# kazuotani14/iLQR

Measured on AMD Instinct MI355X. Metric: iLQR iterations/sec (batch x T timesteps/sec), acrobot T=500 batch=4096, higher is better.
Workload: dtype f64; 1 GPU; acrobot n=4 m=1 T=499 (500 knots), box-QP limits active, FD derivatives + backward/box-QP + 11-alpha search + accept, fixed work; batch_per_gpu=4096, global_batch=4096, T=499, parallelism=batch shards x1, one all_gather of costs

## Files before the change

### ilqr_amd/csrc/backward_hex.hpp

```cpp
#pragma once
#include "solve_tile.hpp"

namespace ilqr {

#ifndef ILQR_COMMIT_ROLLED
#define ILQR_COMMIT_ROLLED 1
#endif

#ifndef ILQR_COMMIT_BATCH
#define ILQR_COMMIT_BATCH 2
#endif
constexpr int kCommitBatch = ILQR_COMMIT_BATCH;

constexpr int HT = 4;
#ifndef ILQR_HEX_SLOT_PAD
#define ILQR_HEX_SLOT_PAD 8
#endif
#ifndef ILQR_HEX_PAIR_PERM
#define ILQR_HEX_PAIR_PERM 1
#endif
#ifndef ILQR_HEX_CAND_T
#define ILQR_HEX_CAND_T 1
#endif
constexpr bool kHexCandT = ILQR_HEX_CAND_T != 0;
#ifndef ILQR_HEX_QUAD_ROLLOUT
#define ILQR_HEX_QUAD_ROLLOUT 1
#endif
constexpr bool kHexQuadRollout = ILQR_HEX_QUAD_ROLLOUT != 0;

template <int NX, int NU, class real, int SLOTS_, bool COMPACT_ = false>
struct HexRing {
  static constexpr bool COMPACT = COMPACT_;
  static constexpr int US = Rec<NX, NU>::SIZE;
  static constexpr int PAIRS = COMPACT ? CompactRec<NX, NU>::PAIRS : (Rec<NX, NU>::SIZE + NU + 1) / 2;
  static constexpr int ROW = 2 * HT;
  static constexpr int PAD = ROW - 2 * TW;
  static constexpr int ELEMS = PAIRS * ROW + ILQR_HEX_SLOT_PAD;
  static constexpr int Z = PAIRS * ROW;
  static_assert(!COMPACT || ILQR_HEX_SLOT_PAD >= ROW, "the compact slot keeps Z in its pad row");
  static_assert(!COMPACT || (NX == 4 && NU == 1), "compact slots: nx = 4, nu = 1");
  static constexpr int SLOTS = SLOTS_;
  static constexpr bool PERM = (ILQR_HEX_PAIR_PERM != 0) && NX == 4 && NU == 1;
  static constexpr int pos(int pair) { return PERM && (!COMPACT || pair < 8) ? hex_pair_pos(pair) : pair; }
};

constexpr int kHexKnotsPerRound = 64 / HT;
constexpr int kHexFullSlots = 24;
template <int NX, int NU, class real, bool COMPACT>
struct HexRingSize {
  using Full = HexRing<NX, NU, real, kHexFullSlots, false>;
  static constexpr int TERM = COMPACT ? ((NX + NX * NX) / 2) * Full::ROW : 0;
  static constexpr int SLOTS = COMPACT ? (kHexFullSlots * Full::ELEMS - TERM) / HexRing<NX, NU, real, 1, COMPACT>::ELEMS : kHexFullSlots;
  static constexpr int LEAD = SLOTS - kHexKnotsPerRound - 1;
  static_assert(SLOTS > LEAD + kHexKnotsPerRound - 1 && LEAD >= 1, "a round must not reach a slot the chain has not left");
  static_assert(SLOTS * HexRing<NX, NU, real, 1, COMPACT>::ELEMS + TERM <= kHexFullSlots * Full::ELEMS, "the pair's records fit the bytes of 24 full slots");
};

template <class real, int N>
struct HexTerm {
  alignas(16) real term[N];
};
template <class real>
struct HexTerm<real, 0> {
  static constexpr real* term = nullptr;
};

template <class real, int NX, int NU, bool COMPACT = false>
struct HexPair : HexTerm<real, HexRingSize<NX, NU, real, COMPACT>::TERM> {
  using Size = HexRingSize<NX, NU, real, COMPACT>;
  using RS = HexRing<NX, NU, real, Size::SLOTS, COMPACT>;
  static constexpr int LEAD = Size::LEAD;
  alignas(16) real ring[RS::SLOTS * RS::ELEMS];
  int rounds_done;
  int consumer_at;
  int passes_started;
  unsigned long long pass_lanes;
};

template <class P>
struct HexGate {
  static constexpr bool kRing = true;
  P& sh;
  const int T, nrounds, N;
  int pass = -1, have = 0;
  int g_next = 0, slot_next = 0, slot_cur = 0;
  __device__ __forceinline__ HexGate(P& s, int T_) : sh(s), T(T_), nrounds((T_ + 1 + kHexKnotsPerRound - 1) / kHexKnotsPerRound), N(nrounds * kHexKnotsPerRound) {}
  __device__ __forceinline__ void begin_pass() {
    pass++;
    have = pass * N;
    g_next = pass * N;
    slot_next = g_next % P::RS::SLOTS;
    __hip_atomic_store(&sh.pass_lanes, __ballot(1), __ATOMIC_RELAXED, __HIP_MEMORY_SCOPE_WORKGROUP);
    __hip_atomic_store(&sh.passes_started, pass + 1, __ATOMIC_RELEASE, __HIP_MEMORY_SCOPE_WORKGROUP);
  }
  __device__ __forceinline__ int slot(int) const { return slot_cur; }
  __device__ __forceinline__ void wait(int) {
    const int G = g_next++;
    slot_cur = slot_next;
    slot_next = (slot_next + 1 == P::RS::SLOTS) ? 0 : slot_next + 1;
    __hip_atomic_store(&sh.consumer_at, G, __ATOMIC_RELAXED, __HIP_MEMORY_SCOPE_WORKGROUP);
    if (G < have) return;
    const int round = pass * nrounds + (G - pass * N) / kHexKnotsPerRound;
    while (__hip_atomic_load(&sh.rounds_done, __ATOMIC_ACQUIRE, __HIP_MEMORY_SCOPE_WORKGROUP) <= round) __builtin_amdgcn_s_sleep(1);
    have = pass * N + ((G - pass * N) / kHexKnotsPerRound + 1) * kHexKnotsPerRound;
  }
  __device__ __forceinline__ void finish() {
    __hip_atomic_store(&sh.consumer_at, 0x3fffffff, __ATOMIC_RELAXED, __HIP_MEMORY_SCOPE_WORKGROUP);
    __hip_atomic_store(&sh.passes_started, -1, __ATOMIC_RELEASE, __HIP_MEMORY_SCOPE_WORKGROUP);
  }
};

__device__ __forceinline__ int hex_first(unsigned long long bal, int t4) {
  return __builtin_ctzll(((bal >> t4) & 0x000F000F000F000Full) | 0x8000000000000000ull);
}
__device__ __forceinline__ void qp1_search_hex(QP1StateT<double>& q, int j, int t4, double step_j0, const double* __restrict__ lds_steps) {
  const double t_x1 = clamp_of(q.x + step_j0 * q.search, q.lo, q.hi);
  const double t_v1 = qp1_value(q, t_x1);
  const bool t_pass = !qp1_armijo_fails(q, t_v1, step_j0);
  const int pp = hex_first(__ballot(t_pass), t4);
  const bool success = pp < 52;
  const int jw = success ? (((pp >> 4) << 2) | (pp & 3)) : 0;
#ifdef ILQR_EXP_NO_STEP_LDS
  q.step = jw == 0 ? 1.0 : 0.6;
#else
  q.step = lds_steps[jw];
#endif
  q.x1 = clamp_of(q.x + q.step * q.search, q.lo, q.hi);
  q.v1 = qp1_value(q, q.x1);
  bool more = p_and(!success, !q.early);
  if (__builtin_expect(__ballot(more) == 0ull, 1)) return;
  {
    const bool stuck = p_and(j >= 1, t_x1 == q.x);
    const int qs = hex_first(__ballot(p_and(stuck, more)), t4);
    if (p_and(more, qs < 52)) {
      q.ls_failed = true;
      more = false;
    }
    if (__ballot(more) == 0ull) return;
  }
  for (int base = 16;; base += 16) {
    const int kn = base + j;
    const double my_step = lds_steps[kn < 104 ? kn : 103];
    const double my_x1 = qp1_trial(q, my_step);
    const double my_v1 = qp1_value(q, my_x1);
    const bool pass = !qp1_armijo_fails(q, my_v1, my_step);
    const bool stuck = p_or(my_step < kMinStep, my_x1 == q.x);
    const int qp = hex_first(__ballot(p_and(pass, more)), t4), qs = hex_first(__ballot(p_and(stuck, more)), t4);
    if (more) {
      if (qp < qs) {
        q.step = lds_steps[base + (((qp >> 4) << 2) | (qp & 3))];
        q.x1 = qp1_trial(q, q.step);
        q.v1 = qp1_value(q, q.x1);
        more = false;
      } else if (qs < 52) {
        q.ls_failed = true;
        more = false;
      }
    }
    if (__ballot(more) == 0ull) return;
  }
}

template <class RS>
__device__ __forceinline__ int hex_pos_rt(int pair) { return RS::pos(pair); }

template <class real>
struct HexStep {
  typedef real pair_t __attribute__((ext_vector_type(2)));
  real F, cxx_rc, cxx_cr, fu_r, cx_r, cxu_r, cxu_c;
  pair_t tail, uw;
};

template <class M, class Gate, class RS>
__device__ __forceinline__ void backward_hex(const BatchViewT<typename M::real>& v, const M& model, const SolverParams& sp, int mode, int tile, int sub,
                                             int lane, const double* __restrict__ lds_steps, Gate& gate, const typename M::real* __restrict__ ring,
                                             const typename M::real* __restrict__ term ) {
  using real = typename M::real;
  using creal = double;
  static_assert(M::NX == 4 && M::NU == 1, "hex chain: nx = 4, nu = 1");
  using R = Rec<4, 1>;
  typedef real real2_t __attribute__((ext_vector_type(2)));
  const int r_ = lane >> 4, t_ = (lane >> 2) & 3, c_ = lane & 3, j16 = 4 * r_ + c_;
  const int t4 = 4 * t_;
  const int l = sub * HT + t_;
  const int b = tile * TW + l;
  if (b >= v.B) return;
  if (mode == 1 && v.status[b] != 0) return;
  const int T = v.T;
  double lambda = v.lambda[b], dlambda = v.dlambda[b];
  const real* __restrict__ ust = v.us + tidx(tile, 0, 0, l, T, 1);
  real* __restrict__ kt = v.kff + tidx(tile, 0, 0, l, T, 1);
  real* __restrict__ Kt = v.Kfb + tidx(tile, 0, 0, l, T, 4);
  typedef const __attribute__((address_space(3))) real lds_cd;
  typedef const __attribute__((address_space(3))) real2_t lds_cd2;
  const creal step_j0 = lds_steps[j16];
  auto mm = [](creal a, creal bb) __attribute__((always_inline)) { return __builtin_amdgcn_mfma_f64_4x4x4f64(a, bb, 0.0, 0, 0, 0); };

  auto load = [&](int t, HexStep<real>& d) __attribute__((always_inline)) {
    gate.wait(t);
    lds_cd* r = (lds_cd*)(ring + gate.slot(t) * RS::ELEMS + t_ * 2);
    auto pair = [&](int e) { return *(lds_cd2*)(r + RS::pos(e >> 1) * RS::ROW); };
    auto one = [&](int e) { return r[hex_pos_rt<RS>(e >> 1) * RS::ROW + (e & 1)]; };
    if constexpr (RS::COMPACT) {
      using C = CompactRec<4, 1>;
      d.F = one(C::FX + r_ + 4 * c_);
      d.fu_r = one(C::FU + r_);
      d.cxx_rc = d.cxx_cr = d.cx_r = d.cxu_r = d.cxu_c = r[RS::Z];
      d.tail = pair(C::CU);
      d.uw = pair(C::US);
      return;
    }
    d.F = one(R::FX + r_ + 4 * c_);
    d.cxx_rc = one(R::CXX + r_ + 4 * c_);
    d.cxx_cr = one(R::CXX + c_ + 4 * r_);
    d.fu_r = one(R::FU + r_);
    d.cx_r = one(R::CX + r_);
    d.cxu_r = one(R::CXU + r_);
    d.cxu_c = one(R::CXU + c_);
    d.tail = pair(R::CU);
    d.uw = pair(RS::US);
  };

  int diverge = 0;
  bool done = false;
  double dV0 = 0, dV1 = 0, gacc = 0;
  auto one_pass = [&]() __attribute__((always_inline)) {
    gate.begin_pass();
    creal V, RVx, kprev;
    const creal lam_r = (creal)lambda;
    {
      gate.wait(T);
      if constexpr (RS::COMPACT) {
        using C = CompactRec<4, 1>;
        lds_cd* r = (lds_cd*)(term + t_ * 2);
        RVx = (creal)r[((C::TERM_CX + r_) >> 1) * RS::ROW + ((C::TERM_CX + r_) & 1)];
        V = (creal)r[((C::TERM_CXX + r_ + 4 * c_) >> 1) * RS::ROW + ((C::TERM_CXX + r_ + 4 * c_) & 1)];
      } else {
      lds_cd* r = (lds_cd*)(ring + gate.slot(T) * RS::ELEMS + t_ * 2);
      RVx = (creal)r[hex_pos_rt<RS>((R::CX + r_) >> 1) * RS::ROW + ((R::CX + r_) & 1)];
      V = (creal)r[hex_pos_rt<RS>((R::CXX + r_ + 4 * c_) >> 1) * RS::ROW + ((R::CXX + r_ + 4 * c_) & 1)];
      }
    }
    kprev = (creal)kt[(unsigned)((T - 1) * TW)];
    __builtin_amdgcn_s_waitcnt(0x0F70);
    dV0 = dV1 = 0;
    diverge = 0;
    gacc = 0;
    real* __restrict__ Kt_i = Kt + (unsigned)(((T - 1) * 4 + c_) * TW);
    real* __restrict__ kt_i = kt + (unsigned)((T - 1) * TW);

    auto step = [&](int i, const HexStep<real>& raw, HexStep<real>& nxt) -> bool {
      const creal F = (creal)raw.F, Rfu = (creal)raw.fu_r;
      const creal cu = (creal)raw.tail.x, cuu = (creal)raw.tail.y, us = (creal)raw.uw.x, usw = (creal)raw.uw.y;
      const creal W = mm(V, F);
      const creal wv = mm(V, Rfu);
      const creal aQu = mm(Rfu, RVx);
      const creal aQx = mm(F, RVx);
      const creal Tm = mm(F, W);
      const creal Tt = mm(W, F);
      const creal aQuu = mm(Rfu, wv);
      const creal aQux_c = mm(Rfu, W);
      const creal aQux_r = mm(W, Rfu);
      const creal Qxx_rc = (creal)raw.cxx_rc + Tm, Qxx_cr = (creal)raw.cxx_cr + Tt;
      const creal Qx_r = (creal)raw.cx_r + aQx;
      const creal Qu = cu + aQu;
      const creal Qux_c = (creal)raw.cxu_c + aQux_c, Qux_r = (creal)raw.cxu_r + aQux_r;
      const creal Quu = cuu + aQuu, QuuF = (cuu + lam_r) + aQuu;
      const creal lo = (creal)model.u_min[0] - us, hi = (creal)model.u_max[0] - us;
      __builtin_amdgcn_sched_barrier(0);
      if (i >= 1) load(i - 1, nxt);
      __builtin_amdgcn_sched_barrier(0);
      creal x;
      int free0;
      creal minv;
      QP1StateT<creal> q1;
      qp1_begin<false>(QuuF, Qu, kprev, lo, hi, q1, false);
      qp1_search_hex(q1, j16, t4, step_j0, lds_steps);
      bool goes_on;
      bool ok = qp1_finish_ok(q1, x, free0, minv, goes_on);
      if (goes_on)
        ok = qp1_continue(
                 q1, [&](QP1StateT<creal>& qs) __attribute__((always_inline)) { qp1_search_hex(qs, j16, t4, step_j0, lds_steps); }, x, free0) >= 1;
      if (!ok) diverge = i;
      const creal k_scale = free0 ? -minv : creal(0);
      const creal K_r = k_scale * Qux_r, K_c = k_scale * Qux_c;
      creal d0 = 0, d1 = 0;
      {
        d0 += x * Qu;
        creal rq = 0;
        rq += (creal(0.5) * x) * Quu;
        d1 += rq * x;
      }
      creal T1_r, T1_c;
      {
        creal acc = 0;
        acc += K_r * Quu;
        T1_r = acc;
      }
      {
        creal acc = 0;
        acc += K_c * Quu;
        T1_c = acc;
      }
      creal Vxn_r, Vn_rc, Vn_cr;
      {
        creal t1 = 0, t2 = 0, t3 = 0;
        t1 += T1_r * x;
        t2 += K_r * Qu;
        t3 += Qux_r * x;
        Vxn_r = ((Qx_r + t1) + t2) + t3;
      }
      {
        creal u1 = 0, u2 = 0, u3 = 0;
        u1 += T1_r * K_c;
        u2 += K_r * Qux_c;
        u3 += Qux_r * K_c;
        Vn_rc = ((Qxx_rc + u1) + u2) + u3;
      }
      {
        creal u1 = 0, u2 = 0, u3 = 0;
        u1 += T1_c * K_r;
        u2 += K_c * Qux_r;
        u3 += Qux_c * K_r;
        Vn_cr = ((Qxx_cr + u1) + u2) + u3;
      }
      V = creal(0.5) * (Vn_rc + Vn_cr);
      RVx = Vxn_r;
      if (ok) {
        dV0 += (double)d0;
        dV1 += (double)d1;
        gacc += (double)(abs_of(x) * usw);
        kprev = (creal)(real)x;
        Kt_i[0] = (real)K_c;
        kt_i[0] = (real)x;
      }
      Kt_i -= 4 * TW;
      kt_i -= TW;
      return ok;
    };

    HexStep<real> A, Bd;
    int i = T - 1;
    load(i, A);
    while (true) {
      if (!step(i, A, Bd)) break;
      if (--i < 0) break;
      if (!step(i, Bd, A)) break;
      if (--i < 0) break;
    }
  };

  while (true) {
    one_pass();
    if (mode == 0) {
      done = (diverge == 0);
      break;
    }
    if (diverge != 0) {
      dlambda = raised_dlambda(dlambda, sp);
      lambda = raised_lambda(lambda, dlambda, sp);
      if (lambda > sp.lambda_max) break;
      continue;
    }
    done = true;
    break;
  }

  double acc = gacc;
  if (!done) {
    __builtin_amdgcn_fence(__ATOMIC_RELEASE, "workgroup");
    __builtin_amdgcn_s_waitcnt(0);
    acc = 0;
    for (int t0 = 0; t0 < T; t0 += 8) {
      real kv[8], uv[8];
#pragma unroll
      for (int jj = 0; jj < 8; jj++) {
        const int t = (t0 + jj < T) ? t0 + jj : T - 1;
        kv[jj] = kt[(size_t)t * TW];
        uv[jj] = ust[(size_t)t * TW];
      }
#pragma unroll
      for (int jj = 0; jj < 8; jj++) {
        const real mx = abs_of(kv[jj]) / (abs_of(uv[jj]) + 1);
        if (t0 + jj < T) acc += (double)mx;
      }
    }
  }
  const double gnorm = acc / T;
  if (j16 == 0) {
    v.dV[b] = dV0;
    v.dV[v.Bp + b] = dV1;
    v.diverge[b] = diverge;
    v.backpass_done[b] = done ? 1 : 0;
    v.gnorm[b] = gnorm;
    if (mode == 1) {
      v.lambda[b] = lambda;
      v.dlambda[b] = dlambda;
      if (!sp.fixed_work && gnorm < sp.tol_grad && lambda < kLambdaConverged) {
        v.status[b] = 1;
        v.iters[b] += 1;
      }
    }
  }
}

template <class M, class MFD, class P>
__device__ __forceinline__ void sweep_backward_hex(const BatchViewT<typename M::real>& v, const M& model, const MFD& fdm, const SolverParams& sp, int mode,
                                                   int force, int tile, P* pairs, const double* __restrict__ lds_steps, int role) {
  using RS = typename P::RS;
  const int lane = threadIdx.x & 63;
  if (threadIdx.x < 4) {
    pairs[threadIdx.x].rounds_done = 0;
    pairs[threadIdx.x].consumer_at = 0;
    pairs[threadIdx.x].passes_started = 0;
  }
  __syncthreads();
  const int T = v.T;
  P& sh = pairs[role & 3];
  if (role < 4) {
    __builtin_amdgcn_s_setprio(3);
    HexGate<P> gate(sh, T);
    backward_hex<M, decltype(gate), RS>(v, model, sp, mode, tile, role, lane, lds_steps, gate, sh.ring, sh.term);
    gate.finish();
    __builtin_amdgcn_s_setprio(0);
  } else {
    const int sub = role - 4;
    const int lp = lane & (HT - 1), ks = lane >> 2;
    const int l = sub * HT + lp;
    const int nrounds = (T + 1 + kHexKnotsPerRound - 1) / kHexKnotsPerRound, N = nrounds * kHexKnotsPerRound;
    for (int pass = 0;; pass++) {
      unsigned long long lanes = ~0ull;
      if (pass > 0) {
        int started;
        while ((started = __hip_atomic_load(&sh.passes_started, __ATOMIC_ACQUIRE, __HIP_MEMORY_SCOPE_WORKGROUP)) >= 0 && started <= pass)
          __builtin_amdgcn_s_sleep(8);
        if (started < 0) break;
        lanes = __hip_atomic_load(&sh.pass_lanes, __ATOMIC_RELAXED, __HIP_MEMORY_SCOPE_WORKGROUP);
      }
      const bool mine = (lanes >> (4 * lp)) & 1ull;
      for (int r = 0; r < nrounds; r++) {
        const int j0 = r * kHexKnotsPerRound, G0 = pass * N + j0;
        while (G0 > __hip_atomic_load(&sh.consumer_at, __ATOMIC_RELAXED, __HIP_MEMORY_SCOPE_WORKGROUP) + P::LEAD) __builtin_amdgcn_s_sleep(4);
        const int started = __hip_atomic_load(&sh.passes_started, __ATOMIC_RELAXED, __HIP_MEMORY_SCOPE_WORKGROUP);
        if ((started < 0) | (started > pass + 1)) break;
        const int t = T - (j0 + ks);
        if (t >= 0 && (pass == 0 || mine)) {
          typename M::real* rs = sh.ring + ((G0 + ks) % RS::SLOTS) * RS::ELEMS + lp * 2;
          if constexpr (RS::COMPACT) {
            if (t == T) rs = sh.term + lp * 2;
          }
          derivatives_of_knot<M, true, MFD, RS::PAD, RS::PERM, RS::COMPACT>(v, model, fdm, force, nullptr, tile, t, l, rs, true);
        }
        __builtin_amdgcn_s_waitcnt(0xC07F);
        if (lane == 0) __hip_atomic_store(&sh.rounds_done, pass * nrounds + r + 1, __ATOMIC_RELEASE, __HIP_MEMORY_SCOPE_WORKGROUP);
      }
    }
  }
}

template <class M, bool CANDT = false>
__device__ __forceinline__ void commit_tile_chunks(const BatchViewT<typename M::real>& v, const M& model, const int* commit_of_lane , int tile) {
  using real = typename M::real;
  constexpr int NX = M::NX, NU = M::NU;
  static_assert(!CANDT || (NX == 4 && NU == 1 && CT == 8 && CG == 4), "grouped candidates: nx = 4, nu = 1");
  static_assert(HT == kQuad, "a chain wavefront rolls out its own sub-tile");
  const int T = v.T;
  const real dt = (real)v.dt;
  const int ntask = v.nch * TW;
  struct Task {
    int l, c;
    real x[NX], uq[CT][NU];
  };
  auto load = [&](int task, Task& k) __attribute__((always_inline)) {
    k.l = 0;
    k.c = -1;
    if (task < 0) return;
    const int l = task & (TW - 1), c = task >> 4;
    const int b = tile * TW + l;
    const int ci = (b < v.B) ? commit_of_lane[l] : -1;
    if (ci < 0) return;
    k.l = l;
    k.c = c;
    const int ta = ci * v.ntiles + tile;
    real* const x = k.x;
    real(*const uq)[NU] = k.uq;
    if constexpr (CANDT) {
      typedef real real4v __attribute__((ext_vector_type(4)));
      const real4v xv = *reinterpret_cast<const real4v*>(v.cand_x + cand_g_x(ta, c, l, v.nch, NX));
      x[0] = xv.x;
      x[1] = xv.y;
      x[2] = xv.z;
      x[3] = xv.w;
      const real4v u0 = *reinterpret_cast<const real4v*>(v.cand_u + cand_g_u(ta, 2 * c, l, T));
      const real4v u1 = *reinterpret_cast<const real4v*>(v.cand_u + cand_g_u(ta, 2 * c + 1, l, T));
      uq[0][0] = u0.x;
      uq[1][0] = u0.y;
      uq[2][0] = u0.z;
      uq[3][0] = u0.w;
      uq[4][0] = u1.x;
      uq[5][0] = u1.y;
      uq[6][0] = u1.z;
      uq[7][0] = u1.w;
    } else {
#pragma unroll
    for (int i = 0; i < NX; i++) x[i] = v.cand_x[tidx(ta, c, i, l, v.nch, NX)];
#pragma unroll
    for (int q = 0; q < CT; q++) {
      const int tq = (c * CT + q < T) ? c * CT + q : T - 1;
#pragma unroll
      for (int jj = 0; jj < NU; jj++) uq[q][jj] = v.cand_u[tidx(ta, tq, jj, l, T, NU)];
    }
    }
  };
  auto steps = [&](Task& k) __attribute__((always_inline)) {
    if (k.c < 0) return;
    const int l = k.l, c = k.c;
    real* const x = k.x;
    real(*const uq)[NU] = k.uq;
#if ILQR_COMMIT_ROLLED
#pragma unroll 1
    for (int q = 0; q < CT; q++) {
      const int t = c * CT + q;
      if (t > T) break;
#pragma unroll
      for (int i = 0; i < NX; i++) v.xs[tidx(tile, t, i, l, T + 1, NX)] = x[i];
      if (t < T) {
#pragma unroll
        for (int jj = 0; jj < NU; jj++) v.us[tidx(tile, t, jj, l, T, NU)] = uq[0][jj];
        if (q + 1 < CT) {
          real x1[NX];
          integrate_dynamics(model, x, uq[0], dt, x1);
#pragma unroll
          for (int i = 0; i < NX; i++) x[i] = x1[i];
        }
      }
#pragma unroll
      for (int qq = 0; qq + 1 < CT; qq++)
#pragma unroll
        for (int jj = 0; jj < NU; jj++) uq[qq][jj] = uq[qq + 1][jj];
    }
#else
#pragma unroll
    for (int q = 0; q < CT; q++) {
      const int t = c * CT + q;
      if (t <= T) {
#pragma unroll
        for (int i = 0; i < NX; i++) v.xs[tidx(tile, t, i, l, T + 1, NX)] = x[i];
        if (t < T) {
#pragma unroll
          for (int jj = 0; jj < NU; jj++) v.us[tidx(tile, t, jj, l, T, NU)] = uq[q][jj];
          if (q + 1 < CT) {
            real x1[NX];
            integrate_dynamics(model, x, uq[q], dt, x1);
#pragma unroll
            for (int i = 0; i < NX; i++) x[i] = x1[i];
          }
        }
      }
    }
#endif
  };
  for (int first = ntask - 1 - (int)threadIdx.x; first >= 0; first -= kCommitBatch * (int)blockDim.x) {
    Task k[kCommitBatch];
#pragma unroll
    for (int j = 0; j < kCommitBatch; j++) load(first - j * (int)blockDim.x, k[j]);
#pragma unroll
    for (int j = 0; j < kCommitBatch; j++) steps(k[j]);
  }
}

template <class M, class MFD>
__global__ __launch_bounds__(512) __attribute__((amdgpu_waves_per_eu(2, 2))) void k_solve_hex(BatchViewT<typename M::real> v, M model, MFD fdm, AlphaSet alphas,
                                                                                                 SolverParams sp, int n_iters, int force,
                                                                                                 int* __restrict__ commit_idx, int commit_pending,
                                                                                                 long long* __restrict__ phase_ticks) {
  using real = typename M::real;
  using P = HexPair<real, M::NX, M::NU, state_free_running_cost<M>::value>;
  __shared__ P pairs[4];
  __shared__ double steps[104];
  __shared__ double lds_cost[NALPHA * TW];
  __shared__ int tile_running;
  __shared__ int simd_count[4];
  __shared__ int lds_commit[TW];
  if (threadIdx.x < 4) simd_count[threadIdx.x] = 0;
  load_step_table(steps);
  const int wave = (int)(threadIdx.x >> 6);
  int role = wave;
  {
    const int simd = hw_simd_id();
    int slot = 0;
    if ((threadIdx.x & 63) == 0) slot = atomicAdd(&simd_count[simd], 1);
    slot = __shfl(slot, 0, 64);
    __syncthreads();
    if (simd_count[0] == 2 && simd_count[1] == 2 && simd_count[2] == 2 && simd_count[3] == 2) role = simd + 4 * slot;
  }
  const int rwave = kHexQuadRollout ? ((role < 4) ? role : 4) : ((role < 3) ? role : 3);
  const int tile = blockIdx.x;
  constexpr int kShareReals = 4 * ((2 * M::NU + M::NU * M::NX + M::NX + 3) / 4) * TW;
  static_assert(kShareReals <= (int)(sizeof(pairs[0].ring) / sizeof(real)), "a pair's ring holds a wavefront's rollout rows");
  long long t_sweep = 0, t_roll = 0, t0 = 0;
#ifdef ILQR_HEX_SECTIONS
  long long t_sweep_last = 0;
#endif
  const bool timing = (phase_ticks != nullptr) & (threadIdx.x == 0);
  const long long c_begin = timing ? clock64() : 0, w_begin = timing ? wall_clock64() : 0;
  if (commit_pending) {
    commit_tile_chunks<M>(v, model, commit_idx + tile * TW, tile);
    phase_barrier();
  }
  int it = 0;
  for (; it < n_iters; it++) {
    if (timing) t0 = wall_clock64();
    sweep_backward_hex<M, MFD, P>(v, model, fdm, sp, 1, force, tile, pairs, steps, role);
    phase_barrier();
    if (timing) {
      const long long t1 = wall_clock64();
#ifdef ILQR_HEX_SECTIONS
      t_sweep_last = t1 - t0;
#endif
      t_sweep += t1 - t0;
      t0 = t1;
    }
    rollout_tile<M, true, true, kDeepPrefetch<M>, true, true, true, 1, kHexCandT, kHexQuadRollout>(v, model, alphas, NALPHA, v.cost_c, 1, sp, commit_idx, tile, lds_cost, it == n_iters - 1, rwave,
                                               pairs[role & 3].ring);
#ifdef ILQR_HEX_SECTIONS
#define ILQR_HEX_MARK(n)                                   \
    if (ILQR_HEX_SECTIONS == n && timing) {                \
      const long long t1 = wall_clock64();                 \
      t_sweep = t_sweep - t_sweep_last + (t1 - t0);        \
      t0 = t1;                                             \
    }
#else
#define ILQR_HEX_MARK(n)
#endif
    ILQR_HEX_MARK(1)
    if (threadIdx.x < TW) lds_commit[threadIdx.x] = commit_idx[tile * TW + threadIdx.x];
    if (threadIdx.x == 0) tile_running = 0;
    phase_barrier();
    ILQR_HEX_MARK(2)
    commit_tile_chunks<M, kHexCandT>(v, model, lds_commit, tile);
    ILQR_HEX_MARK(3)
    phase_barrier();
    if (timing) t_roll += wall_clock64() - t0;
    if (!sp.fixed_work) {
      const int b = tile * TW + (int)threadIdx.x;
      if (threadIdx.x < TW && b < v.B && v.status[b] == 0) tile_running = 1;
      __syncthreads();
      if (!tile_running) {
        it++;
        break;
      }
    }
  }
  if (timing) {
    phase_ticks[5 * tile + 0] += t_sweep;
    phase_ticks[5 * tile + 1] += t_roll;
    phase_ticks[5 * tile + 2] += it;
    phase_ticks[5 * tile + 3] += clock64() - c_begin;
    phase_ticks[5 * tile + 4] += wall_clock64() - w_begin;
  }
}

}
```

### ilqr_amd/csrc/quad_lanes.hpp

```cpp
#pragma once
#include "common.hpp"

namespace ilqr {

constexpr int kQuad = 4;

constexpr int quad_rollout_lanes(int nalpha) { return kQuad * nalpha; }
constexpr int quad_lane_alpha(int lane) { return lane / kQuad; }
constexpr int quad_lane_q(int lane) { return lane % kQuad; }
constexpr int quad_traj(int s, int q) { return kQuad * s + q; }
constexpr int quad_fetch_row(int lane, int nrows) { return lane / kQuad < nrows ? lane / kQuad : nrows - 1; }

constexpr int rollout_share_slot(int row, int l) { return ((row >> 1) * TW + l) * 2 + (row & 1); }
constexpr int rollout_share_pair(int p, int l) { return (p * TW + l) * 2; }
constexpr int rollout_rows(int nx, int nu) { return 2 * nu + nu * nx + nx; }

enum { ROW_US = 0, ROW_KFF = 1, ROW_KFB = 2, ROW_XS = 3 };
struct RowSource {
  int array, elem, E, S;
};
constexpr RowSource rollout_row_source(int row, int nx, int nu, int T) {
  return row < nu                 ? RowSource{ROW_US, row, nu, T}
         : row < 2 * nu           ? RowSource{ROW_KFF, row - nu, nu, T}
         : row < 2 * nu + nu * nx ? RowSource{ROW_KFB, row - 2 * nu, nu * nx, T}
                                  : RowSource{ROW_XS, row - 2 * nu - nu * nx, nx, T + 1};
}
constexpr size_t rollout_row_elem(const RowSource& r, int tile, int tt, int l) {
  return ((((size_t)tile * r.S) * r.E + r.elem) * TW + l) + (size_t)tt * r.E * TW;
}

}
```

### ilqr_amd/csrc/rollout.hpp

```cpp
#pragma once
#include "layout.hpp"
#include "quad_lanes.hpp"

namespace ilqr {

template <class View, class CostOf>
__device__ __forceinline__ void accept_one(const View& v, const SolverParams& sp, int b, CostOf cost_of,
                                           int* __restrict__ commit_idx, bool count_running = true) {
  if (b >= v.Bp) return;
  int commit = -1;
  if (b < v.B && v.status[b] == 0) {
    double lambda = v.lambda[b], dlambda = v.dlambda[b];
    const double cost_s = v.cost[b];
    bool fwd = false;
    double new_cost = 0, dcost = 0;
    int acc = -1;
    if (v.backpass_done[b]) {
      const double dV0 = v.dV[b], dV1 = v.dV[v.Bp + b];
      for (int a = 0; a < NALPHA; a++) {
        const double alpha = kAlpha[a];
        new_cost = cost_of(a);
        dcost = cost_s - new_cost;
        double expected;
        {
#pragma clang fp contract(off)
          expected = -alpha * (dV0 + alpha * dV1);
        }
        double z;
        if (expected > 0)
          z = dcost / expected;
        else
          z = (double)((0.0 < dcost) - (dcost < 0.0));
        if (z > sp.z_min) {
          fwd = true;
          acc = a;
          break;
        }
      }
    }
    int status = 0;
    if (fwd) {
      dlambda = fmin(dlambda / sp.lambda_factor, 1 / sp.lambda_factor);
      lambda = lambda * dlambda * (lambda > sp.lambda_min ? 1.0 : 0.0);
      v.cost[b] = new_cost;
      v.flg_change[b] = 1;
      commit = acc;
      if (!sp.fixed_work && dcost < sp.tol_fun) status = 2;
    } else {
      dlambda = fmax(dlambda * sp.lambda_factor, sp.lambda_factor);
      lambda = fmax(lambda * dlambda, sp.lambda_min);
      v.flg_change[b] = 0;
      if (!sp.fixed_work && lambda > sp.lambda_max) status = 3;
    }
    v.lambda[b] = lambda;
    v.dlambda[b] = dlambda;
    v.alpha_idx[b] = acc;
    const int it = v.iters[b] + 1;
    v.iters[b] = it;
    if (status == 0 && !sp.fixed_work && it >= sp.max_iter) status = 4;
    v.status[b] = status;
    if (status == 0 && count_running) atomicAdd(v.n_running, 1);
  }
  commit_idx[b] = commit;
}
template <class real>
__global__ void k_accept(BatchViewT<real> v, SolverParams sp, int* __restrict__ commit_idx) {
  const int b = blockIdx.x * blockDim.x + threadIdx.x;
  accept_one(v, sp, b, [&](int a) { return v.cost_c[(size_t)a * v.Bp + b]; }, commit_idx);
}

struct AlphaSet {
  double a[NALPHA];
};

#ifndef ILQR_ROLLOUT_UNCLAMPED_FETCH
#define ILQR_ROLLOUT_UNCLAMPED_FETCH 1
#endif
constexpr int kRolloutFetchSlack = 8;
constexpr size_t rollout_fetch_slack_elems(int nx, int nu) { return (size_t)kRolloutFetchSlack * nu * nx * TW; }
template <class M>
constexpr int kDeepPrefetch = (M::NU * M::NX + M::NX + 2 * M::NU <= 10) ? 8 : 4;

constexpr int CG = 4;
static_assert(CT % CG == 0, "a chunk of the commit is a whole number of control groups");
__host__ __device__ inline int cand_groups(int T) { return (T + CT + CG - 1) / CG; }
__host__ __device__ inline size_t cand_g_u(int ta, int grp, int l, int T) { return (((size_t)ta * cand_groups(T) + grp) * TW + l) * CG; }
__host__ __device__ inline size_t cand_g_x(int ta, int c, int l, int nch, int NX) { return (((size_t)ta * nch + c) * TW + l) * NX; }
template <class M, bool GAINS, bool CAND, int PD, bool ACCEPT, bool SHARE = false, bool NOFIX = false, int NG = 1, bool CANDT = false, bool QUAD = false>
__device__ __forceinline__ void rollout_tile(const BatchViewT<typename M::real>& v, const M& model, const AlphaSet& alphas, int n_alpha,
                                             double* __restrict__ cost_out, int mode, const SolverParams& sp,
                                             int* __restrict__ commit_idx, int tile, double* lds_cost, bool count_running = true, int rwave = -1,
                                             typename M::real* share = nullptr) {
  using real = typename M::real;
  constexpr int NX = M::NX, NU = M::NU;
  static_assert(NG == 1 || (SHARE && GAINS && !ACCEPT), "several alpha groups per wavefront: the shared-row rollout of the wide tiles");
  static_assert(!QUAD || (SHARE && GAINS && NG == 1 && quad_rollout_lanes(NALPHA) <= 64 && kQuad * rollout_rows(NX, NU) <= quad_rollout_lanes(NALPHA)),
                "quad rollouts: every alpha of four trajectories in one wavefront, whose lanes also fetch the quad's rows");
  static_assert(!CANDT || (CAND && SHARE && GAINS && NU == 1 && NX == 4 && PD % CG == 0), "grouped candidates: the matrix-core kernel's rollouts (nx = 4, nu = 1)");
  const int wave = (rwave >= 0) ? rwave : (int)(threadIdx.x >> 6);
  const int lane = threadIdx.x & 63;
  const int l = QUAD ? quad_traj(wave & 3, quad_lane_q(lane)) : lane & (TW - 1);
  const bool idle = QUAD && lane >= quad_rollout_lanes(NALPHA);
  const int a_sub = lane >> 4;
  const int b = tile * TW + l;
  int a[NG];
  bool active[NG];
  bool any_active = false;
  const bool eligible = (b < v.B) && (mode != 1 || (v.status[b < v.B ? b : 0] == 0 && v.backpass_done[b < v.B ? b : 0]));
#pragma unroll
  for (int g = 0; g < NG; g++) {
    a[g] = QUAD ? quad_lane_alpha(lane) : (wave + g) * 4 + a_sub;
    active[g] = eligible && (a[g] < n_alpha) && (!QUAD || wave < 4);
    any_active = any_active || active[g];
  }
  const bool run = (SHARE && GAINS) ? (__ballot(any_active) != 0ull) : any_active;
  if (!ACCEPT && !run) return;
  if (run && !idle) {
  const int T = v.T;
  real alpha[NG];
#pragma unroll
  for (int g = 0; g < NG; g++) alpha[g] = (real)alphas.a[a[g] < NALPHA ? a[g] : NALPHA - 1];
  const real dt = (real)v.dt;

  real x[NG][NX];
#pragma unroll
  for (int i = 0; i < NX; i++) {
    const real x0i = v.x0[tidx(tile, 0, i, l, 1, NX)];
#pragma unroll
    for (int g = 0; g < NG; g++) x[g][i] = x0i;
  }
  double total[NG];
#pragma unroll
  for (int g = 0; g < NG; g++) total[g] = 0;

  struct StepIn {
    real u[NU], k[GAINS ? NU : 1], K[GAINS ? NU * NX : 1], xnom[GAINS ? NX : 1];
  };
  auto load_step = [&](int t, StepIn& d) __attribute__((always_inline)) {
    t = (t < T) ? t : T - 1;
#pragma unroll
    for (int j = 0; j < NU; j++) d.u[j] = v.us[tidx(tile, t, j, l, T, NU)];
    if (GAINS) {
#pragma unroll
      for (int j = 0; j < NU; j++) d.k[j] = v.kff[tidx(tile, t, j, l, T, NU)];
#pragma unroll
      for (int e = 0; e < NU * NX; e++) d.K[e] = v.Kfb[tidx(tile, t, e, l, T, NU * NX)];
#pragma unroll
      for (int i = 0; i < NX; i++) d.xnom[i] = v.xs[tidx(tile, t, i, l, T + 1, NX)];
    }
  };
  int ta_store[NG];
#pragma unroll
  for (int g = 0; g < NG; g++) ta_store[g] = ((SHARE && CAND && !active[g]) ? NALPHA : a[g]) * v.ntiles + tile;
  typedef real real4v __attribute__((ext_vector_type(4)));
  real pend[NG][CG - 1];
#pragma unroll
  for (int g = 0; g < NG; g++)
#pragma unroll
    for (int q = 0; q < CG - 1; q++) pend[g][q] = 0;
  auto store_group = [&](int g, int t, real last) __attribute__((always_inline)) {
    real4v w;
    w.x = pend[g][0];
    w.y = pend[g][1];
    w.z = pend[g][2];
    w.w = last;
    *reinterpret_cast<real4v*>(v.cand_u + cand_g_u(ta_store[g], t / CG, l, T)) = w;
  };
  auto emit_knot = [&](int g, int t, const real* xx, const real* uu, auto with_u, auto ph) __attribute__((always_inline)) {
    if (SHARE && !CAND && !active[g]) return;
    if constexpr (CANDT) {
      constexpr int p = decltype(ph)::value;
      if (with_u) {
        if constexpr (p == CG - 1)
          store_group(g, t, uu[0]);
        else
          pend[g][p] = uu[0];
      }
      if ((t & (CT - 1)) == 0) {
        real4v w;
        w.x = xx[0];
        w.y = xx[1];
        w.z = xx[2];
        w.w = xx[3];
        *reinterpret_cast<real4v*>(v.cand_x + cand_g_x(ta_store[g], t / CT, l, v.nch, NX)) = w;
      }
    } else if (CAND) {
      const int ta = ta_store[g];
      if (with_u) {
#pragma unroll
        for (int q = 0; q < NU; q++) v.cand_u[tidx(ta, t, q, l, T, NU)] = uu[q];
      }
      if ((t & (CT - 1)) == 0) {
#pragma unroll
        for (int i = 0; i < NX; i++) v.cand_x[tidx(ta, t / CT, i, l, v.nch, NX)] = xx[i];
      }
    } else {
#pragma unroll
      for (int i = 0; i < NX; i++) v.xs[tidx(tile, t, i, l, T + 1, NX)] = xx[i];
      if (with_u) {
#pragma unroll
        for (int q = 0; q < NU; q++) v.us[tidx(tile, t, q, l, T, NU)] = uu[q];
      }
    }
  };
  const WithTrigConsts<M> rmodel(model);
  auto do_step = [&](int t, const StepIn& d, auto ph) __attribute__((always_inline)) {
#pragma unroll
    for (int g = 0; g < NG; g++) {
      real u[NU];
#pragma unroll
      for (int j = 0; j < NU; j++) u[j] = d.u[j];
      if (GAINS) {
#pragma unroll
        for (int j = 0; j < NU; j++) {
          u[j] += d.k[j] * alpha[g];
          real acc = 0;
#pragma unroll
          for (int i = 0; i < NX; i++) acc += d.K[j + NU * i] * (x[g][i] - d.xnom[i]);
          u[j] += acc;
        }
      }
      if (!NOFIX && (sp.fixes & 1)) {
#pragma unroll
        for (int j = 0; j < NU; j++) u[j] = min_of(max_of(u[j], model.u_min[j]), model.u_max[j]);
      }
      emit_knot(g, t, x[g], u, std::true_type(), ph);
      total[g] += (double)model.cost(x[g], u);
      real x1[NX];
      integrate_dynamics(rmodel, x[g], u, dt, x1);
#pragma unroll
      for (int i = 0; i < NX; i++) x[g][i] = x1[i];
    }
  };
  if constexpr (SHARE && GAINS) {
    static_assert(PD % 2 == 0 || PD == 1, "static ring indices");
    static_assert((size_t)PD * NU * NX * TW <= rollout_fetch_slack_elems(NX, NU), "PD knots past the end");
    constexpr int NROWS = 2 * NU + NU * NX + NX;
    static_assert(NROWS == rollout_rows(NX, NU), "quad_lanes.hpp counts the same rows");
    constexpr int NLD = QUAD ? 1 : (NROWS + 3) / 4;
    struct Raw {
      real r[NLD];
    };
    const real* rbase[NLD];
    unsigned rstride[NLD];
#pragma unroll
    for (int j = 0; j < NLD; j++) {
      const int row = QUAD ? quad_fetch_row(lane, NROWS) : (a_sub + 4 * j < NROWS) ? a_sub + 4 * j : NROWS - 1;
      if (row < NU) {
        rbase[j] = v.us + tidx(tile, 0, row, l, T, NU);
        rstride[j] = NU * TW;
      } else if (row < 2 * NU) {
        rbase[j] = v.kff + tidx(tile, 0, row - NU, l, T, NU);
        rstride[j] = NU * TW;
      } else if (row < 2 * NU + NU * NX) {
        rbase[j] = v.Kfb + tidx(tile, 0, row - 2 * NU, l, T, NU * NX);
        rstride[j] = NU * NX * TW;
      } else {
        rbase[j] = v.xs + tidx(tile, 0, row - 2 * NU - NU * NX, l, T + 1, NX);
        rstride[j] = NX * TW;
      }
    }
    auto fetch = [&](int tt, Raw& d) __attribute__((always_inline)) {
#if !ILQR_ROLLOUT_UNCLAMPED_FETCH
      tt = (tt < T) ? tt : T - 1;
#endif
#pragma unroll
      for (int j = 0; j < NLD; j++) d.r[j] = rbase[j][(size_t)tt * rstride[j]];
    };
    typedef real real2_t __attribute__((ext_vector_type(2)));
    constexpr int NPAIR = (NROWS + 1) / 2;
    real* const mine = share + (QUAD ? rollout_share_slot(quad_fetch_row(lane, NROWS), l) : rollout_share_slot(a_sub, l));
    auto put = [&](const Raw& d) __attribute__((always_inline)) {
#pragma unroll
      for (int j = 0; j < NLD; j++) mine[4 * j * TW] = d.r[j];
    };
    const real2_t* const row0 = reinterpret_cast<const real2_t*>(share + rollout_share_pair(0, l));
    auto get = [&](StepIn& d) __attribute__((always_inline)) {
      real rows[2 * NPAIR];
#pragma unroll
      for (int q = 0; q < NPAIR; q++) {
        const real2_t pr = row0[q * TW];
        rows[2 * q] = pr.x;
        rows[2 * q + 1] = pr.y;
      }
#pragma unroll
      for (int j = 0; j < NU; j++) d.u[j] = rows[j];
#pragma unroll
      for (int j = 0; j < NU; j++) d.k[j] = rows[NU + j];
#pragma unroll
      for (int e = 0; e < NU * NX; e++) d.K[e] = rows[2 * NU + e];
#pragma unroll
      for (int i = 0; i < NX; i++) d.xnom[i] = rows[2 * NU + NU * NX + i];
    };
    Raw ring[PD];
#pragma unroll
    for (int d = 0; d < PD; d++) fetch(d, ring[d]);
    StepIn cur, nxt;
    put(ring[0]);
    get(cur);
    auto one = [&](int s_, Raw& free_set, const Raw& next_set, auto ph) __attribute__((always_inline)) {
      put(next_set);
      get(nxt);
      fetch(s_ + PD, free_set);
      do_step(s_, cur, ph);
      cur = nxt;
    };
    int t = 0;
    for (; t + PD <= T; t += PD) {
      static_for<PD>([&](auto dc) __attribute__((always_inline)) {
        constexpr int d = decltype(dc)::value;
        one(t + d, ring[d], ring[(d + 1) % PD], std::integral_constant<int, d % CG>());
      });
    }
    static_for<PD>([&](auto dc) __attribute__((always_inline)) {
      constexpr int d = decltype(dc)::value;
      if (t + d < T) one(t + d, ring[d], ring[(d + 1) % PD], std::integral_constant<int, d % CG>());
    });
  } else {
  StepIn ring[PD];
#pragma unroll
  for (int d = 0; d < PD; d++) load_step(d, ring[d]);
  int t = 0;
  for (; t + PD <= T; t += PD) {
#pragma unroll
    for (int d = 0; d < PD; d++) {
      do_step(t + d, ring[d], std::integral_constant<int, 0>());
      load_step(t + d + PD, ring[d]);
    }
  }
  for (; t < T; t++) {
    StepIn cur;
    load_step(t, cur);
    do_step(t, cur, std::integral_constant<int, 0>());
  }
  }
#pragma unroll
  for (int g = 0; g < NG; g++) {
    {
      real uz[NU];
#pragma unroll
      for (int q = 0; q < NU; q++) uz[q] = 0;
      emit_knot(g, T, x[g], uz, std::false_type(), std::integral_constant<int, 0>());
      if constexpr (CANDT) {
        if (T % CG) store_group(g, T - 1, pend[g][CG - 2]);
      }
    }
    total[g] += (double)model.final_cost(x[g]);
    if (active[g]) {
      cost_out[(size_t)a[g] * v.Bp + b] = total[g];
      if (ACCEPT) lds_cost[a[g] * TW + l] = total[g];
    }
  }
  }
  if constexpr (ACCEPT) {
    __syncthreads();
    if (threadIdx.x < TW)
      accept_one(v, sp, tile * TW + (int)threadIdx.x, [&](int aa) { return lds_cost[aa * TW + threadIdx.x]; }, commit_idx, count_running);
  }
}

template <class M, bool GAINS, bool CAND, int PD = 4, bool ACCEPT = false>
__global__ __launch_bounds__(192) void k_rollout(BatchViewT<typename M::real> v, M model, AlphaSet alphas, int n_alpha,
                                                 double* __restrict__ cost_out, int mode, SolverParams sp,
                                                 int* __restrict__ commit_idx) {
  __shared__ double lds_cost[ACCEPT ? NALPHA * TW : 1];
  rollout_tile<M, GAINS, CAND, PD, ACCEPT>(v, model, alphas, n_alpha, cost_out, mode, sp, commit_idx, (int)blockIdx.x, lds_cost);
}

template <class M, bool CANDT = false>
__device__ __forceinline__ void candidate_knot(const BatchViewT<typename M::real>& v, const M& model, int a, int tile, int t, int l,
                                               typename M::real* x, typename M::real* u) {
  using real = typename M::real;
  constexpr int NX = M::NX, NU = M::NU;
  const int T = v.T, ta = a * v.ntiles + tile, c = t / CT, off = t - c * CT;
#pragma unroll
  for (int i = 0; i < NX; i++) x[i] = CANDT ? v.cand_x[cand_g_x(ta, c, l, v.nch, NX) + i] : v.cand_x[tidx(ta, c, i, l, v.nch, NX)];
  real uq[CT][NU];
#pragma unroll
  for (int q = 0; q < CT; q++) {
    const int tq = (c * CT + q < T) ? c * CT + q : T - 1;
#pragma unroll
    for (int j = 0; j < NU; j++) uq[q][j] = CANDT ? v.cand_u[cand_g_u(ta, tq / CG, l, T) + tq % CG] : v.cand_u[tidx(ta, tq, j, l, T, NU)];
  }
#pragma unroll
  for (int j = 0; j < NU; j++) u[j] = 0.0;
#pragma unroll
  for (int q = 0; q < CT; q++) {
    if (q < off) {
      real x1[NX];
      integrate_dynamics(model, x, uq[q], (real)v.dt, x1);
#pragma unroll
      for (int i = 0; i < NX; i++) x[i] = x1[i];
    }
    if (q == off && t < T) {
#pragma unroll
      for (int j = 0; j < NU; j++) u[j] = uq[q][j];
    }
  }
}

template <class M, bool CANDT = false>
__global__ void k_unpack_cand(BatchViewT<typename M::real> v, M model, int a, double* __restrict__ xs, double* __restrict__ us) {
  using real = typename M::real;
  constexpr int NX = M::NX, NU = M::NU;
  const int T = v.T;
  const size_t n = (size_t)v.B * (T + 1);
  for (size_t i = (size_t)blockIdx.x * blockDim.x + threadIdx.x; i < n; i += (size_t)gridDim.x * blockDim.x) {
    const int t = (int)(i % (T + 1));
    const int b = (int)(i / (T + 1));
    real x[NX], u[NU];
    candidate_knot<M, CANDT>(v, model, a, b / TW, t, b % TW, x, u);
    if (xs)
      for (int e = 0; e < NX; e++) xs[((size_t)b * (T + 1) + t) * NX + e] = (double)x[e];
    if (us && t < T)
      for (int e = 0; e < NU; e++) us[((size_t)b * T + t) * NU + e] = (double)u[e];
  }
}

}
```

Measured before the change: 4.546 billion trajectory-timesteps/s.

## Pair rollout and accept waves per quad to replace block-wide tail barriers

After the backward sweep, each quad's rollout wavefront now hands its alpha costs to a partner wavefront through LDS generation counters instead of a block-wide __syncthreads. The partner prefetches the per-trajectory accept state (status, lambda, cost, dV, iters) while it waits, runs the line-search accept for its four trajectories, and publishes the commit indices. Each pair of wavefronts then commits its own quad's chunks. This removes the whole-block barriers between rollout, accept and commit so quads can proceed independently, at the cost of spin-wait loops and a more intricate per-role schedule that relies on the fixed role-to-SIMD mapping.

```diff
diff --git a/ilqr_amd/csrc/backward_hex.hpp b/ilqr_amd/csrc/backward_hex.hpp
--- a/ilqr_amd/csrc/backward_hex.hpp
+++ b/ilqr_amd/csrc/backward_hex.hpp
@@ -27,6 +27,10 @@
 #define ILQR_HEX_QUAD_ROLLOUT 1
 #endif
 constexpr bool kHexQuadRollout = ILQR_HEX_QUAD_ROLLOUT != 0;
+#ifndef ILQR_HEX_PAIR_TAIL
+#define ILQR_HEX_PAIR_TAIL 1
+#endif
+constexpr bool kHexPairTail = ILQR_HEX_PAIR_TAIL != 0 && kHexQuadRollout && kHexCandT;
 
 template <int NX, int NU, class real, int SLOTS_, bool COMPACT_ = false>
 struct HexRing {
@@ -458,15 +462,17 @@
   }
 }
 
-template <class M, bool CANDT = false>
-__device__ __forceinline__ void commit_tile_chunks(const BatchViewT<typename M::real>& v, const M& model, const int* commit_of_lane , int tile) {
+template <class M, bool CANDT = false, bool PAIR = false>
+__device__ __forceinline__ void commit_tile_chunks(const BatchViewT<typename M::real>& v, const M& model, const int* commit_of_lane , int tile,
+                                                   int sub = 0, int pt = 0) {
   using real = typename M::real;
   constexpr int NX = M::NX, NU = M::NU;
   static_assert(!CANDT || (NX == 4 && NU == 1 && CT == 8 && CG == 4), "grouped candidates: nx = 4, nu = 1");
   static_assert(HT == kQuad, "a chain wavefront rolls out its own sub-tile");
   const int T = v.T;
   const real dt = (real)v.dt;
-  const int ntask = v.nch * TW;
+  const int ntask = PAIR ? quad_commit_tasks(v.nch) : v.nch * TW;
+  const int me = PAIR ? pt : (int)threadIdx.x, nthr = PAIR ? kPairThreads : (int)blockDim.x;
   struct Task {
     int l, c;
     real x[NX], uq[CT][NU];
@@ -475,7 +481,7 @@
     k.l = 0;
     k.c = -1;
     if (task < 0) return;
-    const int l = task & (TW - 1), c = task >> 4;
+    const int l = PAIR ? quad_traj(sub, quad_commit_q(task)) : task & (TW - 1), c = PAIR ? quad_commit_chunk(task) : task >> 4;
     const int b = tile * TW + l;
     const int ci = (b < v.B) ? commit_of_lane[l] : -1;
     if (ci < 0) return;
@@ -560,13 +566,45 @@
     }
 #endif
   };
-  for (int first = ntask - 1 - (int)threadIdx.x; first >= 0; first -= kCommitBatch * (int)blockDim.x) {
+  for (int first = ntask - 1 - me; first >= 0; first -= kCommitBatch * nthr) {
     Task k[kCommitBatch];
 #pragma unroll
-    for (int j = 0; j < kCommitBatch; j++) load(first - j * (int)blockDim.x, k[j]);
+    for (int j = 0; j < kCommitBatch; j++) load(first - j * nthr, k[j]);
 #pragma unroll
     for (int j = 0; j < kCommitBatch; j++) steps(k[j]);
   }
+}
+
+struct HexTailSync {
+  int costs_at[4];
+  int accepts_at[4];
+};
+template <class M>
+__device__ __forceinline__ void hex_pair_tail(const BatchViewT<typename M::real>& v, const M& model, const AlphaSet& alphas, const SolverParams& sp,
+                                              int* __restrict__ commit_idx, int tile, double* lds_cost, int* lds_commit, HexTailSync& sync, int it,
+                                              bool count_running, int role, typename M::real* share) {
+  const int lane = threadIdx.x & 63, s = role & 3, gen = it + 1;
+  if (role < 4) {
+    rollout_tile<M, true, true, kDeepPrefetch<M>, true, true, true, 1, true, true, true>(v, model, alphas, NALPHA, v.cost_c, 1, sp, commit_idx, tile, lds_cost,
+                                                                                         count_running, role, share);
+    __hip_atomic_store(&sync.costs_at[s], gen, __ATOMIC_RELEASE, __HIP_MEMORY_SCOPE_WORKGROUP);
+    while (__hip_atomic_load(&sync.accepts_at[s], __ATOMIC_ACQUIRE, __HIP_MEMORY_SCOPE_WORKGROUP) < gen) __builtin_amdgcn_s_sleep(1);
+  } else {
+    const int l = quad_traj(s, lane & (kQuad - 1)), b = tile * TW + l;
+    const bool accepts = lane < kQuad;
+    AcceptPreloaded in;
+    if (accepts && b < v.B) in.fetch(v, b);
+    while (__hip_atomic_load(&sync.costs_at[s], __ATOMIC_ACQUIRE, __HIP_MEMORY_SCOPE_WORKGROUP) < gen) __builtin_amdgcn_s_sleep(8);
+    if (accepts) {
+      int commit = -1;
+      in.commit_ = &commit;
+      accept_one(v, sp, b, [&](int a) { return lds_cost[a * TW + l]; }, commit_idx, count_running, in);
+      lds_commit[l] = commit;
+    }
+    __hip_atomic_store(&sync.accepts_at[s], gen, __ATOMIC_RELEASE, __HIP_MEMORY_SCOPE_WORKGROUP);
+  }
+  __builtin_amdgcn_fence(__ATOMIC_ACQUIRE, "agent");
+  commit_tile_chunks<M, true, true>(v, model, lds_commit, tile, s, (role < 4 ? 0 : 64) + lane);
 }
 
 template <class M, class MFD>
@@ -582,7 +620,9 @@
   __shared__ int tile_running;
   __shared__ int simd_count[4];
   __shared__ int lds_commit[TW];
+  __shared__ HexTailSync tail_sync;
   if (threadIdx.x < 4) simd_count[threadIdx.x] = 0;
+  if (threadIdx.x < 4) tail_sync.costs_at[threadIdx.x] = tail_sync.accepts_at[threadIdx.x] = 0;
   load_step_table(steps);
   const int wave = (int)(threadIdx.x >> 6);
   int role = wave;
@@ -621,6 +661,10 @@
       t_sweep += t1 - t0;
       t0 = t1;
     }
+    if constexpr (kHexPairTail) {
+      if (threadIdx.x == 0) tile_running = 0;
+      hex_pair_tail<M>(v, model, alphas, sp, commit_idx, tile, lds_cost, lds_commit, tail_sync, it, it == n_iters - 1, role, pairs[role & 3].ring);
+    } else {
     rollout_tile<M, true, true, kDeepPrefetch<M>, true, true, true, 1, kHexCandT, kHexQuadRollout>(v, model, alphas, NALPHA, v.cost_c, 1, sp, commit_idx, tile, lds_cost, it == n_iters - 1, rwave,
                                                pairs[role & 3].ring);
 #ifdef ILQR_HEX_SECTIONS
@@ -640,6 +684,7 @@
     ILQR_HEX_MARK(2)
     commit_tile_chunks<M, kHexCandT>(v, model, lds_commit, tile);
     ILQR_HEX_MARK(3)
+    }
     phase_barrier();
     if (timing) t_roll += wall_clock64() - t0;
     if (!sp.fixed_work) {
diff --git a/ilqr_amd/csrc/quad_lanes.hpp b/ilqr_amd/csrc/quad_lanes.hpp
--- a/ilqr_amd/csrc/quad_lanes.hpp
+++ b/ilqr_amd/csrc/quad_lanes.hpp
@@ -10,6 +10,12 @@
 constexpr int quad_lane_q(int lane) { return lane % kQuad; }
 constexpr int quad_traj(int s, int q) { return kQuad * s + q; }
 constexpr int quad_fetch_row(int lane, int nrows) { return lane / kQuad < nrows ? lane / kQuad : nrows - 1; }
+
+constexpr int kPairThreads = 128;
+constexpr int quad_commit_tasks(int nch) { return kQuad * nch; }
+constexpr int quad_commit_q(int task) { return task % kQuad; }
+constexpr int quad_commit_chunk(int task) { return task / kQuad; }
+constexpr int quad_commit_task(int ntask, int pt, int j) { return ntask - 1 - pt - kPairThreads * j; }
 
 constexpr int rollout_share_slot(int row, int l) { return ((row >> 1) * TW + l) * 2 + (row & 1); }
 constexpr int rollout_share_pair(int p, int l) { return (p * TW + l) * 2; }
diff --git a/ilqr_amd/csrc/rollout.hpp b/ilqr_amd/csrc/rollout.hpp
--- a/ilqr_amd/csrc/rollout.hpp
+++ b/ilqr_amd/csrc/rollout.hpp
@@ -4,19 +4,56 @@
 
 namespace ilqr {
 
-template <class View, class CostOf>
+struct AcceptFromMemory {
+  template <class View> __device__ __forceinline__ int status(const View& v, int b) const { return v.status[b]; }
+  template <class View> __device__ __forceinline__ double lambda(const View& v, int b) const { return v.lambda[b]; }
+  template <class View> __device__ __forceinline__ double dlambda(const View& v, int b) const { return v.dlambda[b]; }
+  template <class View> __device__ __forceinline__ double cost(const View& v, int b) const { return v.cost[b]; }
+  template <class View> __device__ __forceinline__ int backpass_done(const View& v, int b) const { return v.backpass_done[b]; }
+  template <class View> __device__ __forceinline__ double dV0(const View& v, int b) const { return v.dV[b]; }
+  template <class View> __device__ __forceinline__ double dV1(const View& v, int b) const { return v.dV[v.Bp + b]; }
+  template <class View> __device__ __forceinline__ int iters(const View& v, int b) const { return v.iters[b]; }
+  __device__ __forceinline__ void accepted(int) const {}
+};
+struct AcceptPreloaded {
+  int status_ = 1, backpass_done_ = 0, iters_ = 0;
+  int* commit_ = nullptr;
+  double lambda_ = 0, dlambda_ = 0, cost_ = 0, dV0_ = 0, dV1_ = 0;
+  template <class View>
+  __device__ __forceinline__ void fetch(const View& v, int b) {
+    status_ = v.status[b];
+    lambda_ = v.lambda[b];
+    dlambda_ = v.dlambda[b];
+    cost_ = v.cost[b];
+    backpass_done_ = v.backpass_done[b];
+    dV0_ = v.dV[b];
+    dV1_ = v.dV[v.Bp + b];
+    iters_ = v.iters[b];
+  }
+  template <class View> __device__ __forceinline__ int status(const View&, int) const { return status_; }
+  template <class View> __device__ __forceinline__ double lambda(const View&, int) const { return lambda_; }
+  template <class View> __device__ __forceinline__ double dlambda(const View&, int) const { return dlambda_; }
+  template <class View> __device__ __forceinline__ double cost(const View&, int) const { return cost_; }
+  template <class View> __device__ __forceinline__ int backpass_done(const View&, int) const { return backpass_done_; }
+  template <class View> __device__ __forceinline__ double dV0(const View&, int) const { return dV0_; }
+  template <class View> __device__ __forceinline__ double dV1(const View&, int) const { return dV1_; }
+  template <class View> __device__ __forceinline__ int iters(const View&, int) const { return iters_; }
+  __device__ __forceinline__ void accepted(int commit) const { *commit_ = commit; }
+};
+
+template <class View, class CostOf, class In = AcceptFromMemory>
 __device__ __forceinline__ void accept_one(const View& v, const SolverParams& sp, int b, CostOf cost_of,
-                                           int* __restrict__ commit_idx, bool count_running = true) {
+                                          int* __restrict__ commit_idx, bool count_running = true, In in = In()) {
   if (b >= v.Bp) return;
   int commit = -1;
-  if (b < v.B && v.status[b] == 0) {
-    double lambda = v.lambda[b], dlambda = v.dlambda[b];
-    const double cost_s = v.cost[b];
+  if (b < v.B && in.status(v, b) == 0) {
+    double lambda = in.lambda(v, b), dlambda = in.dlambda(v, b);
+    const double cost_s = in.cost(v, b);
     bool fwd = false;
     double new_cost = 0, dcost = 0;
     int acc = -1;
-    if (v.backpass_done[b]) {
-      const double dV0 = v.dV[b], dV1 = v.dV[v.Bp + b];
+    if (in.backpass_done(v, b)) {
+      const double dV0 = in.dV0(v, b), dV1 = in.dV1(v, b);
       for (int a = 0; a < NALPHA; a++) {
         const double alpha = kAlpha[a];
         new_cost = cost_of(a);
@@ -55,13 +92,14 @@
     v.lambda[b] = lambda;
     v.dlambda[b] = dlambda;
     v.alpha_idx[b] = acc;
-    const int it = v.iters[b] + 1;
+    const int it = in.iters(v, b) + 1;
     v.iters[b] = it;
     if (status == 0 && !sp.fixed_work && it >= sp.max_iter) status = 4;
     v.status[b] = status;
     if (status == 0 && count_running) atomicAdd(v.n_running, 1);
   }
   commit_idx[b] = commit;
+  in.accepted(commit);
 }
 template <class real>
 __global__ void k_accept(BatchViewT<real> v, SolverParams sp, int* __restrict__ commit_idx) {
@@ -86,7 +124,7 @@
 __host__ __device__ inline int cand_groups(int T) { return (T + CT + CG - 1) / CG; }
 __host__ __device__ inline size_t cand_g_u(int ta, int grp, int l, int T) { return (((size_t)ta * cand_groups(T) + grp) * TW + l) * CG; }
 __host__ __device__ inline size_t cand_g_x(int ta, int c, int l, int nch, int NX) { return (((size_t)ta * nch + c) * TW + l) * NX; }
-template <class M, bool GAINS, bool CAND, int PD, bool ACCEPT, bool SHARE = false, bool NOFIX = false, int NG = 1, bool CANDT = false, bool QUAD = false>
+template <class M, bool GAINS, bool CAND, int PD, bool ACCEPT, bool SHARE = false, bool NOFIX = false, int NG = 1, bool CANDT = false, bool QUAD = false, bool QACCEPT = false>
 __device__ __forceinline__ void rollout_tile(const BatchViewT<typename M::real>& v, const M& model, const AlphaSet& alphas, int n_alpha,
                                              double* __restrict__ cost_out, int mode, const SolverParams& sp,
                                              int* __restrict__ commit_idx, int tile, double* lds_cost, bool count_running = true, int rwave = -1,
@@ -96,6 +134,7 @@
   static_assert(NG == 1 || (SHARE && GAINS && !ACCEPT), "several alpha groups per wavefront: the shared-row rollout of the wide tiles");
   static_assert(!QUAD || (SHARE && GAINS && NG == 1 && quad_rollout_lanes(NALPHA) <= 64 && kQuad * rollout_rows(NX, NU) <= quad_rollout_lanes(NALPHA)),
                 "quad rollouts: every alpha of four trajectories in one wavefront, whose lanes also fetch the quad's rows");
+  static_assert(!QACCEPT || (ACCEPT && QUAD), "accept per quad: the quad rollouts");
   static_assert(!CANDT || (CAND && SHARE && GAINS && NU == 1 && NX == 4 && PD % CG == 0), "grouped candidates: the matrix-core kernel's rollouts (nx = 4, nu = 1)");
   const int wave = (rwave >= 0) ? rwave : (int)(threadIdx.x >> 6);
   const int lane = threadIdx.x & 63;
@@ -352,7 +391,7 @@
     }
   }
   }
-  if constexpr (ACCEPT) {
+  if constexpr (ACCEPT && !QACCEPT) {
     __syncthreads();
     if (threadIdx.x < TW)
       accept_one(v, sp, tile * TW + (int)threadIdx.x, [&](int aa) { return lds_cost[aa * TW + threadIdx.x]; }, commit_idx, count_running);
```

After: 4.556 billion trajectory-timesteps/s (median of 4 runs). About the same (+0.2%).
